# COSIMA/cice4

Measured on AMD Instinct MI355X. Metric: EVP subcycles/sec, higher is better.
Workload: dtype f64; 1 GPU; gx1-size 320x384 rectangular synthetic grid, full ice cover, ncat=5, ndte=120; nx_global=320, ny_global=384, ndte=120, decomposition=1x1 j-slabs, one block per GPU, subcycles_in_the_most_common_launch=120, metrics_recomputed_from_HTN_HTE=True, active_T_cells=121980, active_U_cells=121280

## Files before the change

cice4_amd/csrc/evp.hip:

```cpp
#include "evp.h"

#include <algorithm>
#include <array>
#include <cmath>
#include <cstdio>
#include <cstdlib>
#include <chrono>
#include <cstring>
#include <thread>

namespace cice {

using namespace K;

#ifdef CICE4_AMD_AUSCOM
__constant__ double cosw = 1.0, sinw = 0.0, dragw = dragio * rhow;
__constant__ int ocnslope = 0;

void evp_set_namelist(double cosw_, double sinw_, double dragio_, int use_ocnslope) {
  const double dragw_ = dragio_ * rhow;
  const int os = use_ocnslope != 0;
  CICE_HIP(hipMemcpyToSymbol(HIP_SYMBOL(cosw), &cosw_, 8));
  CICE_HIP(hipMemcpyToSymbol(HIP_SYMBOL(sinw), &sinw_, 8));
  CICE_HIP(hipMemcpyToSymbol(HIP_SYMBOL(dragw), &dragw_, 8));
// ... 89 lines not shown
  const double ssigm1 = (m1 + m3) * p055, ssigm2 = (m2 + m4) * p055;
  const double ssig12n = t1 + t2, ssig12s = t3 + t4, ssig12e = t1 + t4, ssig12w = t2 + t3;
  const double ssig121 = (t1 + t3) * p111, ssig122 = (t2 + t4) * p111;
  const double csigpne = p111 * p1 + ssigp2 + p027 * p3;
  const double csigpnw = p111 * p2 + ssigp1 + p027 * p4;
  const double csigpsw = p111 * p3 + ssigp2 + p027 * p1;
  const double csigpse = p111 * p4 + ssigp1 + p027 * p2;
  const double csigmne = p111 * m1 + ssigm2 + p027 * m3;
  const double csigmnw = p111 * m2 + ssigm1 + p027 * m4;
  const double csigmsw = p111 * m3 + ssigm2 + p027 * m1;
  const double csigmse = p111 * m4 + ssigm1 + p027 * m2;
  const double csig12ne = p222 * t1 + ssig122 + p055 * t3;
  const double csig12nw = p222 * t2 + ssig121 + p055 * t4;
  const double csig12sw = p222 * t3 + ssig122 + p055 * t1;
  const double csig12se = p222 * t4 + ssig121 + p055 * t2;
  const double str12ew = p5 * Dxt * (p333 * ssig12e + p166 * ssig12w);
  const double str12we = p5 * Dxt * (p333 * ssig12w + p166 * ssig12e);
  const double str12ns = p5 * Dyt * (p333 * ssig12n + p166 * ssig12s);
  const double str12sn = p5 * Dyt * (p333 * ssig12s + p166 * ssig12n);
  double strp_tmp = p25 * Dyt * (p333 * ssigpn + p166 * ssigps);
  double strm_tmp = p25 * Dyt * (p333 * ssigmn + p166 * ssigms);
  o.str[0] = -strp_tmp - strm_tmp - str12ew + Dxhy * (-csigpne + csigmne) + Dyhx * csig12ne;
  o.str[1] = strp_tmp + strm_tmp - str12we + Dxhy * (-csigpnw + csigmnw) + Dyhx * csig12nw;
  strp_tmp = p25 * Dyt * (p333 * ssigps + p166 * ssigpn);
  strm_tmp = p25 * Dyt * (p333 * ssigms + p166 * ssigmn);
  o.str[2] = -strp_tmp - strm_tmp + str12ew + Dxhy * (-csigpse + csigmse) + Dyhx * csig12se;
  o.str[3] = strp_tmp + strm_tmp + str12we + Dxhy * (-csigpsw + csigmsw) + Dyhx * csig12sw;
  strp_tmp = p25 * Dxt * (p333 * ssigpe + p166 * ssigpw);
  strm_tmp = p25 * Dxt * (p333 * ssigme + p166 * ssigmw);
  o.str[4] = -strp_tmp + strm_tmp - str12ns - Dyhx * (csigpne + csigmne) + Dxhy * csig12ne;
  o.str[5] = strp_tmp - strm_tmp - str12sn - Dyhx * (csigpse + csigmse) + Dxhy * csig12se;
  strp_tmp = p25 * Dxt * (p333 * ssigpw + p166 * ssigpe);
  strm_tmp = p25 * Dxt * (p333 * ssigmw + p166 * ssigme);
  o.str[6] = -strp_tmp + strm_tmp + str12ns - Dyhx * (csigpnw + csigmnw) + Dxhy * csig12nw;
  o.str[7] = strp_tmp - strm_tmp + str12sn - Dyhx * (csigpsw + csigmsw) + Dxhy * csig12sw;
}

__device__ __forceinline__ void water_of(double uo, double vo, double fmv, double& wx, double& wy) {
#ifdef CICE4_AMD_AUSCOM
  const double sg = __builtin_signbit(fmv) ? -1.0 : 1.0;
  wx = uo * cosw - vo * sinw * sg;
  wy = vo * cosw + uo * sinw * sg;
#else
  (void)fmv;
  wx = uo * cosw - vo * sinw;
  wy = vo * cosw + uo * sinw;
#endif
}

struct StepuOut {
  double u, v, strintx, strinty, taux, tauy;
};

__device__ __forceinline__ void stepu_cell(double uold, double vold, double Aiu, double Uocn,
                                           double Vocn, double Waterx, double Watery, double Forcex,
                                           double Forcey, double Umassdtei, double Fm, double Uarear,
                                           double sx, double sy, StepuOut& o) {
  const double du = Uocn - uold, dv = Vocn - vold;
  const double vrel = Aiu * dragw * sqrt(du * du + dv * dv);
  o.taux = vrel * Waterx;
  o.tauy = vrel * Watery;
  const double cca = Umassdtei + vrel * cosw;
#ifdef CICE4_AMD_AUSCOM
  const double ccb = Fm < 0.0 ? Fm - vrel * sinw : Fm + vrel * sinw;
#else
  const double ccb = Fm + vrel * sinw;
#endif
  const double ab2 = cca * cca + ccb * ccb;
  o.strintx = Uarear * sx;
  o.strinty = Uarear * sy;
  const double cc1 = o.strintx + Forcex + o.taux + Umassdtei * uold;
  const double cc2 = o.strinty + Forcey + o.tauy + Umassdtei * vold;
  o.u = (cca * cc1 + ccb * cc2) / ab2;
  o.v = (cca * cc2 - ccb * cc1) / ab2;
}

}

struct SubArgs {
  EvpScalars sc;
  int nx, ny, tiles_x, tiles_y, nblocks;
  int diag_jmin;
  int carry_top;
  int ew_cyclic;
  size_t n;
  const int32_t* __restrict__ ring_slot;
  const int32_t* __restrict__ fwd;
  const int32_t* __restrict__ blk;
  const int32_t* __restrict__ icetmask;
  const int32_t* __restrict__ iceumask;
  const double* __restrict__ u_in;
  const double* __restrict__ v_in;
  double* __restrict__ u_out;
  double* __restrict__ v_out;
  const double* __restrict__ sig_in;
  double* __restrict__ sig_out;
  const double* sig_in_p[12];
  double* sig_out_p[12];
  const double *__restrict__ dxt, *__restrict__ dyt, *__restrict__ dxhy, *__restrict__ dyhx,
      *__restrict__ cxp, *__restrict__ cyp, *__restrict__ cxm, *__restrict__ cym,
      *__restrict__ tarear, *__restrict__ tinyarea, *__restrict__ strength;
  const double *__restrict__ HTN, *__restrict__ HTE;
  const double *__restrict__ aiu, *__restrict__ uocn, *__restrict__ vocn, *__restrict__ waterx,
      *__restrict__ watery, *__restrict__ forcex, *__restrict__ forcey, *__restrict__ umassdtei,
      *__restrict__ fm, *__restrict__ uarear;
  double *__restrict__ divu, *__restrict__ rdg_conv, *__restrict__ rdg_shear, *__restrict__ shear,
      *__restrict__ prs_sig, *__restrict__ strintx, *__restrict__ strinty, *__restrict__ strocnx,
      *__restrict__ strocny;
};

namespace {


__device__ __forceinline__ double up1(double x) {
  int lo = __double2loint(x), hi = __double2hiint(x);
  lo = __builtin_amdgcn_update_dpp(lo, lo, 0x138, 0xf, 0xf, false);
  hi = __builtin_amdgcn_update_dpp(hi, hi, 0x138, 0xf, 0xf, false);
  return __hiloint2double(hi, lo);
}
__device__ __forceinline__ double down1(double x) {
  int lo = __double2loint(x), hi = __double2hiint(x);
  lo = __builtin_amdgcn_update_dpp(lo, lo, 0x130, 0xf, 0xf, false);
  hi = __builtin_amdgcn_update_dpp(hi, hi, 0x130, 0xf, 0xf, false);
  return __hiloint2double(hi, lo);
}

#ifndef SKEW_OPAQUE_STRIDE
#define SKEW_OPAQUE_STRIDE 1
#endif
#ifndef SKEW_TRIM
#define SKEW_TRIM 1
#endif
#ifndef SKEW_LOADPRIO
#define SKEW_LOADPRIO 1
#endif
#ifndef SKEW_TPASS
#define SKEW_TPASS 1
#endif
#ifndef SKEW_WIDE
#define SKEW_WIDE 1
#endif
#if !defined(CICE4_AMD_EXPERIMENTS) || !defined(SKEW_EARLY)
#undef SKEW_EARLY
#define SKEW_EARLY 0
#endif
__device__ __forceinline__ double up1z(double x) {
  int lo = __double2loint(x), hi = __double2hiint(x);
  lo = __builtin_amdgcn_update_dpp(0, lo, 0x138, 0xf, 0xf, true);
  hi = __builtin_amdgcn_update_dpp(0, hi, 0x138, 0xf, 0xf, true);
  return __hiloint2double(hi, lo);
}
__device__ __forceinline__ double down1z(double x) {
  int lo = __double2loint(x), hi = __double2hiint(x);
  lo = __builtin_amdgcn_update_dpp(0, lo, 0x130, 0xf, 0xf, true);
  hi = __builtin_amdgcn_update_dpp(0, hi, 0x130, 0xf, 0xf, true);
  return __hiloint2double(hi, lo);
}

constexpr int TX = 64;

struct UIn {
  double aiu, uocn, vocn, waterx, watery, forcex, forcey, umassdtei, fm, uarear;
};

template <bool DERIVE>
__device__ __forceinline__ void load_uin(const SubArgs& a, size_t q, UIn& x) {
  x.aiu = a.aiu[q]; x.uocn = a.uocn[q]; x.vocn = a.vocn[q];
  if (!DERIVE) {
    x.waterx = a.waterx[q];
    x.watery = a.watery[q];
  }
  x.forcex = a.forcex[q]; x.forcey = a.forcey[q];
  x.umassdtei = a.umassdtei[q]; x.fm = a.fm[q]; x.uarear = a.uarear[q];
  if (DERIVE) water_of(x.uocn, x.vocn, x.fm, x.waterx, x.watery);
}

template <bool LAST>
__device__ __forceinline__ void stepu_store(const SubArgs& a, const UIn& x, size_t q, int i, int j,
                                            int ilo, int ihi, int jlo, int jhi, double uold,
                                            double vold, double sx, double sy) {
  StepuOut r;
  stepu_cell(uold, vold, x.aiu, x.uocn, x.vocn, x.waterx, x.watery, x.forcex, x.forcey, x.umassdtei,
             x.fm, x.uarear, sx, sy, r);
  a.u_out[q] = r.u;
  a.v_out[q] = r.v;
  if (LAST && j >= a.diag_jmin) {
    a.strintx[q] = r.strintx;
    a.strinty[q] = r.strinty;
    a.strocnx[q] = r.taux;
    a.strocny[q] = r.tauy;
  }
  if (a.ring_slot && (i == ilo || i == ihi || j == jlo || j == jhi)) {
    const int slot = a.ring_slot[q];
    if (slot >= 0) {
#pragma unroll
      for (int k = 0; k < 3; ++k) {
        const int d = a.fwd[3 * slot + k];
        if (d >= 0) {
          a.u_out[d] = r.u;
          a.v_out[d] = r.v;
        }
      }
    }
  }
}

template <int W, int R, bool LAST, bool DAMP, bool DERIVE>
__global__ __launch_bounds__(64 * W, 4) void k_subcycle(const SubArgs a) {
// ... 924 lines not shown
    PHASE(2)
    __syncthreads();
    PHASE(3)
  }
  if (!ra) break;
  }
  stamp_at(sa.stamps, 1);
#ifdef CICE4_AMD_STAMPS
  ph_[6] = (long long)__builtin_amdgcn_s_getreg(20 | (31 << 11));
  ph_[7] = (long long)__builtin_amdgcn_s_getreg(4 | (31 << 11));
  if (sa.phases && lx == 0)
    for (int i_ = 0; i_ < 8; ++i_) sa.phases[8 * ((size_t)blockIdx.x * K + k) + i_] = ph_[i_];
#endif
  if (sa.dbg && threadIdx.x == 0) sa.dbg[2 * blockIdx.x + 1] = wall_clock64();
}

constexpr int RES_MAXDEP = 16;
constexpr int RES_NPEER = 8;
constexpr int RES_STRIDE = 32;

struct ResArgs {
  SubArgs a;
  int nsub, last;
  unsigned epoch0;
  unsigned* prog;
  unsigned* abort_flag;
  const int32_t* deps;
  double* xu[2];
  long long spin_ticks;
  const int32_t* rslot;
  const int32_t* rfwd;
  double* pxu[RES_NPEER][2];
  unsigned pn[RES_NPEER];
  unsigned* prp[RES_NPEER];
  const unsigned* rprog;
  const int32_t* pub;
  const int32_t* fslot;
  const int32_t* ffwd;
  const int32_t* ftab;
  double* xraw[2];
  unsigned* prog2;
  const int32_t* deps2;
  long long* stamps;
  long long* phases;
  int prio_mode;
  int prio_div;
  int prio_top;
  const int32_t* tile_map;
  const int32_t* src;
  void* xg;
  unsigned xg_half;
  void* xgr;
  int poll_delay, poll_sleep;
  int fake_ew;
};
enum { F_LO = 1, F_HI = 2, F_NEG = 4, F_SELF = 8, F_MIRROR = 16 };

__device__ __forceinline__ double ld_agent(const double* base, unsigned off) {
  return __hip_atomic_load((double*)((char*)const_cast<double*>(base) + off), __ATOMIC_RELAXED, __HIP_MEMORY_SCOPE_AGENT);
}
__device__ __forceinline__ void st_agent(double* base, unsigned off, double v) {
  __hip_atomic_store((double*)((char*)base + off), v, __ATOMIC_RELAXED, __HIP_MEMORY_SCOPE_AGENT);
}

__device__ __forceinline__ double ld_sys(const double* base, unsigned off) {
  return __hip_atomic_load((double*)((char*)const_cast<double*>(base) + off), __ATOMIC_RELAXED, __HIP_MEMORY_SCOPE_SYSTEM);
}
__device__ __forceinline__ void st_sys(double* base, unsigned off, double v) {
  __hip_atomic_store((double*)((char*)base + off), v, __ATOMIC_RELAXED, __HIP_MEMORY_SCOPE_SYSTEM);
}

typedef unsigned u32x4 __attribute__((ext_vector_type(4)));
__device__ __forceinline__ void st_gran(__amdgpu_buffer_rsrc_t rs, unsigned off, unsigned soff, double x, unsigned tag) {
  u32x4 g;
  g.x = (unsigned)__double2loint(x); g.y = tag; g.z = (unsigned)__double2hiint(x); g.w = tag;
  __builtin_amdgcn_raw_buffer_store_b128(g, rs, (int)off, (int)soff, 16);
  asm volatile("s_nop 1" : : "v"(g) : "memory");
}
__device__ __forceinline__ u32x4 ld_gran(__amdgpu_buffer_rsrc_t rs, unsigned off, unsigned soff) {
  return __builtin_amdgcn_raw_buffer_load_b128(rs, (int)off, (int)soff, 16);
}
#ifdef CICE4_AMD_STAMPS
__device__ __forceinline__ unsigned gran_tag(unsigned epoch) { return (epoch << 16) | ((unsigned)wall_clock64() & 0xffffu); }
__device__ __forceinline__ bool gran_ok(const u32x4& a, const u32x4& b, unsigned tag) {
  return ((a.y ^ tag) >> 16) == 0 && a.w == a.y && b.y == a.y && b.w == a.y;
}
#else
__device__ __forceinline__ unsigned gran_tag(unsigned epoch) { return epoch; }
__device__ __forceinline__ bool gran_ok(const u32x4& a, const u32x4& b, unsigned tag) {
  return a.y == tag && a.w == tag && b.y == tag && b.w == tag;
}
#endif
__device__ __forceinline__ double gran_val(const u32x4& a) { return __hiloint2double((int)a.z, (int)a.x); }

__global__ __launch_bounds__(1024) void k_res_choose_map(int nt, int tiles_x, int tiles_y, int W, int nx, int ny, int per_xcd,
                                                         int force, const int32_t* __restrict__ blk,
                                                         const int32_t* __restrict__ tmk, const int32_t* __restrict__ umk,
                                                         int32_t* __restrict__ out, unsigned* __restrict__ cover_word) {
  __shared__ int s_ice[1024];
  __shared__ int s_cnt[2][256];
  __shared__ int s_max[2];
  const int t = threadIdx.x;
  if (t < 256) s_cnt[0][t] = s_cnt[1][t] = 0;
  if (t < 2) s_max[t] = 0;
  int ice = 0;
  if (t < nt) {
    const int per_blk = tiles_x * tiles_y, b = t / per_blk, rem = t - b * per_blk, tyi = rem / tiles_x, txi = rem - tyi * tiles_x;
// ... 125 lines not shown
          for (int c = 0; c < 4; ++c) rf[c] = r.rfwd[4 * rs + c];
        }
      }
#pragma unroll
      for (int c = 0; c < 4; ++c) s_rfd[w][c][lx] = rf[c];
      edge = edge || rf[0] >= 0;
    }
    if (FOLD) {
      if (uown) {
        const int rs = r.fslot[q];
        if (rs >= 0) {
#pragma unroll
          for (int c = 0; c < 4; ++c) rfr[c] = r.ffwd[4 * rs + c];
        }
      }
      edge = edge || rfr[0] >= 0;
    }
  }
  const bool topc = FOLD && uown && j == jhi;
  const bool toptile = FOLD && j0 + (W - 2) >= jhi;
  int fpad = -1, fmode = 0;
  if (topc) {
    fpad = r.ftab[2 * q];
    fmode = r.ftab[2 * q + 1];
    edge = true;
  }
  const bool rghost = PEER && ok && !uown && r.rslot[q] == -2;
  bool need_f = false, need_s = false;
  const unsigned qg = (unsigned)q * 32u, nxg = (unsigned)nx * 32u;
  unsigned offA = qg, offB = qg - nxg;
  bool nA = false, nB = false;
  int lw = -1, lq = -1;
  bool lw_a = false, lq_a = false;
  if (GRAN) {
    auto produced = [&](size_t cell) { return r.src[cell] >= 0; };
    need_f = foreign && produced(q);
    need_s = south_h && produced(q - nx);
    nA = need_f;
    nB = need_s;
    const bool nw_ = west_h && produced(q - 1), nq_ = west_h && produced(q - nx - 1);
    const unsigned q0g = (unsigned)__builtin_amdgcn_readfirstlane((int)qg);
    const unsigned long long want_w = __ballot(nw_), want_q = __ballot(nq_);
    auto lend = [&](unsigned off, int& lane, bool& in_a) {
      const unsigned long long fa = __ballot(!nA && lx != 0), fb = __ballot(!nB && lx != 0);
      in_a = fa != 0;
      lane = (int)__builtin_ctzll(in_a ? fa : (fb ? fb : 1ull));
      if (lx == lane && lane != 0) {
        if (in_a) { offA = off; nA = true; }
        else { offB = off; nB = true; }
      }
    };
    if (want_w) lend(q0g - 32u, lw, lw_a);
    if (want_q) lend(q0g - nxg - 32u, lq, lq_a);
    if (r.fake_ew && w > 0 && w < W - 1) {
      nA = nB = false;
      lw = lq = -1;
    }
  }
  StressOut o;
  StepuOut ro{};

  s_uv[w][0][lx] = un;
  s_uv[w][1][lx] = vn;
  __syncthreads();
  if (PEER) {
    const unsigned begun = r.epoch0 + 1u;
    if (threadIdx.x == 0)
      __hip_atomic_store(r.prog + (size_t)tile * RES_STRIDE, begun, __ATOMIC_RELAXED, __HIP_MEMORY_SCOPE_AGENT);
    if (threadIdx.x < RES_NPEER && s_pub[threadIdx.x])
      __hip_atomic_store(r.prp[threadIdx.x] + (size_t)tile * RES_STRIDE, begun, __ATOMIC_RELAXED, __HIP_MEMORY_SCOPE_SYSTEM);
  }
  stamp_at(r.stamps, 0);
  PHASE_DECL
  const int gen = r.prio_div > 0 ? min(2, (int)(blockIdx.x >> 3) / r.prio_div) : 0;
  if (!GRAN && r.prio_mode == 1) {
    if (gen == 0) __builtin_amdgcn_s_setprio(3);
    else if (gen == 1) __builtin_amdgcn_s_setprio(2);
    else __builtin_amdgcn_s_setprio(0);
  }
  if constexpr (GRAN) {
#ifndef GRAN_COPIES
#define GRAN_COPIES 2
#endif
    const __amdgpu_buffer_rsrc_t rs = __builtin_amdgcn_make_buffer_rsrc(r.xg, 0, GRAN_COPIES * r.xg_half, 0x00020000);
    const bool prio_work = r.prio_mode >= 5;
    const bool chain_hi = r.prio_mode == 5 && (w == 0 || w >= W - 2);
    auto prio_wait = [&]() { if (prio_work) __builtin_amdgcn_s_setprio(0); };
    auto prio_compute = [&]() {
      if (prio_work) {
        if (chain_hi) __builtin_amdgcn_s_setprio(3);
        else __builtin_amdgcn_s_setprio(2);
      }
    };
    auto wait_row = [&](int* flag, int want) -> bool {
      long long t0 = 0;
      for (int it = 0;; ++it) {
        if (__hip_atomic_load(flag, __ATOMIC_RELAXED, __HIP_MEMORY_SCOPE_WORKGROUP) >= want) break;
        if (it == 0) prio_wait();
        if (__hip_atomic_load(&s_abort, __ATOMIC_RELAXED, __HIP_MEMORY_SCOPE_WORKGROUP)) return false;
        if (it == 0) t0 = wall_clock64();
        else if ((it & 63) == 0 && wall_clock64() - t0 > 2 * r.spin_ticks) {
          if (lx == 0 && __hip_atomic_exchange(r.abort_flag, 1u, __ATOMIC_RELAXED, __HIP_MEMORY_SCOPE_AGENT) == 0u) {
            r.abort_flag[1] = 5u; r.abort_flag[2] = (unsigned)tile; r.abort_flag[3] = 0u;
            r.abort_flag[4] = (unsigned)w; r.abort_flag[5] = (unsigned)want; r.abort_flag[6] = 0u;
          }
          __hip_atomic_store(&s_abort, 1, __ATOMIC_RELAXED, __HIP_MEMORY_SCOPE_WORKGROUP);
          return false;
        }
        __builtin_amdgcn_s_sleep(1);
      }
      asm volatile("" ::: "memory");
      prio_compute();
      return true;
    };
    auto post_row = [&](int* flag, int value) {
      asm volatile("s_waitcnt lgkmcnt(0)" ::: "memory");
      if (lx == 0) __hip_atomic_store(flag, value, __ATOMIC_RELAXED, __HIP_MEMORY_SCOPE_WORKGROUP);
    };
    TRACE_DECL
    const bool chain = w == 0 || w >= W - 2;
    if (r.prio_mode == 1) {
      if (chain) __builtin_amdgcn_s_setprio(3);
      else __builtin_amdgcn_s_setprio(1);
    }
    prio_compute();
#pragma clang loop unroll(disable)
    for (int k = 0; k < r.nsub; ++k) {
      const bool lastk = r.last && k == r.nsub - 1;
      if (r.prio_mode == 2) {
        const int p = (k + gen) % 3;
        if (p == 0) __builtin_amdgcn_s_setprio(3);
        else if (p == 1) __builtin_amdgcn_s_setprio(1);
        else __builtin_amdgcn_s_setprio(0);
      } else if (r.prio_mode == 3) {
        int behind = 0, level = 0;
        for (int o = w & 3; o < W - 1; o += 4)
          if (o != w) {
            const int done = __hip_atomic_load(&s_uf[o], __ATOMIC_RELAXED, __HIP_MEMORY_SCOPE_WORKGROUP);
            behind += done < k;
            level += done == k;
          }
        if (behind) __builtin_amdgcn_s_setprio(0);
        else if (level) __builtin_amdgcn_s_setprio(2);
        else __builtin_amdgcn_s_setprio(3);
      } else if (r.prio_mode == 4) {
        const int p = (k + gen) & 3;
        if (p == 0) __builtin_amdgcn_s_setprio(3);
        else if (p == 1) __builtin_amdgcn_s_setprio(2);
        else if (p == 2) __builtin_amdgcn_s_setprio(1);
        else __builtin_amdgcn_s_setprio(0);
      }
      PHASE(7)
      TRACE(0)
      if (w > 0) {
        if (!wait_row(&s_uf[w - 1], k)) return;
        if (!south_h) {
          us = s_uv[w - 1][0][lx];
          vs = s_uv[w - 1][1][lx];
        }
      }
      TRACE(1)
      double uw = up1(un), vw = up1(vn), usw = up1(us), vsw = up1(vs);
      if (lx == 0) {
        uw = uwh;
        vw = vwh;
        usw = uswh;
        vsw = vswh;
      }
#pragma unroll
      for (int c = 0; c < 8; ++c) o.str[c] = c0;
      if (tact) {
        const double Dxt = s_m[w][0][lx], Dyt = s_m[w][1][lx], Dxhy = s_m[w][2][lx], Dyhx = s_m[w][3][lx],
                     Cxp = s_m[w][5][lx], Cyp = s_m[w][6][lx], Cxm = s_m[w][7][lx], Cym = s_m[w][8][lx],
                     Tiny = s_m[w][9][lx];
        stress_cell<true, DAMP>(a.sc, un, uw, usw, us, vn, vw, vsw, vs, Dxt, Dyt, Dxhy, Dyhx, Cxp, Cyp, Cxm, Cym,
                                lastk ? a.tarear[q] : c0, Tiny, s_m[w][4][lx], s, o, lastk);
      }
      const double e1 = down1(o.str[1]), e3 = down1(o.str[3]), e6 = down1(o.str[6]), e7 = down1(o.str[7]);
      if (w > 0) {
        s_edge[w][0][lx] = o.str[2];
        s_edge[w][1][lx] = e3;
        s_edge[w][2][lx] = o.str[5];
        s_edge[w][3][lx] = e7;
      }
      post_row(&s_sf[w], k + 1);
      TRACE(2)
      PHASE(0)
      if (w < W - 1) {
        if (!wait_row(&s_sf[w + 1], k + 1)) return;
        TRACE(3)
        PHASE(1)
        if (uact) {
          const double sx = o.str[0] + e1 + s_edge[w + 1][0][lx] + s_edge[w + 1][1][lx];
          const double sy = o.str[4] + s_edge[w + 1][2][lx] + e6 + s_edge[w + 1][3][lx];
          const double uocn = s_x[w][1][lx], vocn = s_x[w][2][lx];
          double wx, wy;
          water_of(uocn, vocn, s_x[w][6][lx], wx, wy);
          stepu_cell(un, vn, s_x[w][0][lx], uocn, vocn, wx, wy,
                     s_x[w][3][lx], s_x[w][4][lx], s_x[w][5][lx], s_x[w][6][lx], s_x[w][7][lx], sx, sy, ro);
          un = ro.u;
          vn = ro.v;
        }
      }
      const unsigned par = (unsigned)(k & (GRAN_COPIES - 1)) * r.xg_half;
      if constexpr (FOLD) {
        if (__any(topc)) {
          const __amdgpu_buffer_rsrc_t rsr = __builtin_amdgcn_make_buffer_rsrc(r.xgr, 0, 4 * r.xg_half, 0x00020000);
          const unsigned tag2 = gran_tag(r.epoch0 + (unsigned)k + 1u);
          const unsigned par4 = (unsigned)(k & 3) * r.xg_half;
          if (topc) {
            st_gran(rsr, qg, par4, un, tag2);
            st_gran(rsr, qg + 16u, par4, vn, tag2);
          }
          bool pp = topc && fmode != 0 && !(fmode & F_SELF);
          u32x4 p0 = {0u, 0u, 0u, 0u}, p1 = p0;
          if (__any(pp)) {
            prio_wait();
            const long long t0 = wall_clock64();
            int it = 0;
            while (true) {
              if (pp) { p0 = ld_gran(rsr, (unsigned)fpad * 32u, par4); p1 = ld_gran(rsr, (unsigned)fpad * 32u + 16u, par4); }
              if (pp && gran_ok(p0, p1, tag2)) pp = false;
              if (!__any(pp)) break;
              asm volatile("" ::: "memory");
              int bad = __hip_atomic_load(&s_abort, __ATOMIC_RELAXED, __HIP_MEMORY_SCOPE_WORKGROUP);
              if (!bad && (++it & 7) == 0) bad = (int)__hip_atomic_load(r.abort_flag, __ATOMIC_RELAXED, __HIP_MEMORY_SCOPE_AGENT);
              if (!bad && wall_clock64() - t0 > r.spin_ticks) {
                if (lx == (int)__builtin_ctzll(__ballot(pp)) &&
                    __hip_atomic_exchange(r.abort_flag, 1u, __ATOMIC_RELAXED, __HIP_MEMORY_SCOPE_AGENT) == 0u) {
                  r.abort_flag[1] = 6u; r.abort_flag[2] = (unsigned)tile; r.abort_flag[3] = (unsigned)k;
                  r.abort_flag[4] = (unsigned)w; r.abort_flag[5] = (unsigned)lx; r.abort_flag[6] = tag2;
                }
                bad = 1;
              }
              if (__any(bad)) {
                __hip_atomic_store(&s_abort, 1, __ATOMIC_RELAXED, __HIP_MEMORY_SCOPE_WORKGROUP);
                return;
              }
              __builtin_amdgcn_s_sleep(1);
            }
            prio_compute();
          }
          if (topc && fmode) {
            if (fmode & F_SELF) {
              un = -un;
              vn = -vn;
            } else {
              const double pu = gran_val(p0), pv = gran_val(p1);
              if (fmode & F_MIRROR) {
                un = (fmode & F_NEG) ? -pu : pu;
                vn = (fmode & F_NEG) ? -pv : pv;
              } else {
                const double u1 = (fmode & F_LO) ? un : pu, u2 = (fmode & F_LO) ? pu : un;
                const double v1 = (fmode & F_LO) ? vn : pv, v2 = (fmode & F_LO) ? pv : vn;
                const double xu_ = 0.5 * (u1 + (-u2)), xv_ = 0.5 * (v1 + (-v2));
                un = (fmode & F_NEG) ? -xu_ : xu_;
                vn = (fmode & F_NEG) ? -xv_ : xv_;
              }
            }
          }
        }
      }
      if (k + 1 == r.nsub) break;
      const unsigned tag = gran_tag(r.epoch0 + (unsigned)k + 1u);
      if (edge) {
        st_gran(rs, qg, par, un, tag);
        st_gran(rs, qg + 16u, par, vn, tag);
#pragma unroll
        for (int c = 0; c < 3; ++c) {
          const int fd = s_fd[w][c][lx];
          if (fd >= 0) {
            st_gran(rs, (unsigned)fd * 32u, par, un, tag);
            st_gran(rs, (unsigned)fd * 32u + 16u, par, vn, tag);
          }
        }
        if (FOLD) {
#pragma unroll
          for (int c = 0; c < 4; ++c) {
            const int rf = rfr[c];
            if (rf >= 0) {
              const bool neg = (rf >> 30) & 1;
              const unsigned ro = (unsigned)(rf & 0x3fffffff) * 32u;
              st_gran(rs, ro, par, neg ? -un : un, tag);
              st_gran(rs, ro + 16u, par, neg ? -vn : vn, tag);
            }
          }
        }
      }
      s_uv[w][0][lx] = un;
      s_uv[w][1][lx] = vn;
      post_row(&s_uf[w], k + 1);
      TRACE(4)
      PHASE(2)
      bool pa = nA, pb = nB;
      if (__any(pa || pb)) {
        prio_wait();
        const long long t0 = wall_clock64();
        int it = 0;
        for (int d = 0; d < r.poll_delay; ++d) __builtin_amdgcn_s_sleep(8);
        u32x4 a0 = {0u, 0u, 0u, 0u}, a1 = a0, b0 = a0, b1 = a0;
        while (true) {
          if (pa) { a0 = ld_gran(rs, offA, par); a1 = ld_gran(rs, offA + 16u, par); }
          if (pb) { b0 = ld_gran(rs, offB, par); b1 = ld_gran(rs, offB + 16u, par); }
          if (pa && gran_ok(a0, a1, tag)) pa = false;
          if (pb && gran_ok(b0, b1, tag)) pb = false;
          PHASE_COUNT(4, 1)
          if (it == 0) { PHASE(3) }
          if (!__any(pa || pb)) break;
          asm volatile("" ::: "memory");
          int bad = __hip_atomic_load(&s_abort, __ATOMIC_RELAXED, __HIP_MEMORY_SCOPE_WORKGROUP);
          if (!bad && (++it & 7) == 0) bad = (int)__hip_atomic_load(r.abort_flag, __ATOMIC_RELAXED, __HIP_MEMORY_SCOPE_AGENT);
          if (!bad && wall_clock64() - t0 > r.spin_ticks) {
            if (lx == (int)__builtin_ctzll(__ballot(pa || pb)) &&
                __hip_atomic_exchange(r.abort_flag, 1u, __ATOMIC_RELAXED, __HIP_MEMORY_SCOPE_AGENT) == 0u) {
              r.abort_flag[1] = 4u; r.abort_flag[2] = (unsigned)tile; r.abort_flag[3] = (unsigned)k;
              r.abort_flag[4] = (unsigned)w; r.abort_flag[5] = (unsigned)lx | (pa ? 256u : 0u) | (pb ? 512u : 0u);
              r.abort_flag[6] = tag;
            }
            bad = 1;
          }
          if (__any(bad)) {
            __hip_atomic_store(&s_abort, 1, __ATOMIC_RELAXED, __HIP_MEMORY_SCOPE_WORKGROUP);
            return;
          }
          __builtin_amdgcn_s_sleep(1);
          for (int d = 0; d < r.poll_sleep; ++d) __builtin_amdgcn_s_sleep(8);
        }
#ifdef CICE4_AMD_STAMPS
        {
          const unsigned now = (unsigned)wall_clock64() & 0xffffu;
          const unsigned ta = nA ? ((now - a0.y) & 0xffffu) : 0u, tb = nB ? ((now - b0.y) & 0xffffu) : 0u;
          PHASE_COUNT(5, (long long)(ta > tb ? ta : tb))
        }
#endif
        const double au = gran_val(a0), av = gran_val(a1), bu = gran_val(b0), bv = gran_val(b1);
        if (need_f) { un = au; vn = av; }
        if (need_s) { us = bu; vs = bv; }
        if (lw >= 0) {
          const double xu_ = __shfl(lw_a ? au : bu, lw), xv_ = __shfl(lw_a ? av : bv, lw);
          if (lx == 0) { uwh = xu_; vwh = xv_; }
        }
        if (lq >= 0) {
          const double xu_ = __shfl(lq_a ? au : bu, lq), xv_ = __shfl(lq_a ? av : bv, lq);
          if (lx == 0) { uswh = xu_; vswh = xv_; }
        }
        prio_compute();
      }
      TRACE(5)
      PHASE(6)
    }
  } else {
#pragma clang loop unroll(disable)
  for (int k = 0; k < r.nsub; ++k) {
    const bool lastk = r.last && k == r.nsub - 1;
    if (FOLD && toptile && r.prio_top) {
      __builtin_amdgcn_s_setprio(3);
    } else if (r.prio_mode == 2) {
      const int p = (k + gen) % 3;
      if (p == 0) __builtin_amdgcn_s_setprio(3);
      else if (p == 1) __builtin_amdgcn_s_setprio(1);
      else __builtin_amdgcn_s_setprio(0);
    }
    PHASE_DRAIN
    PHASE(7)
    if (!south_h && w > 0) {
      us = s_uv[w - 1][0][lx];
      vs = s_uv[w - 1][1][lx];
    }
    double uw = up1(un), vw = up1(vn), usw = up1(us), vsw = up1(vs);
    if (lx == 0) {
      uw = uwh;
      vw = vwh;
      usw = uswh;
      vsw = vswh;
    }
#pragma unroll
    for (int c = 0; c < 8; ++c) o.str[c] = c0;
    if (tact) {
      const double Dxt = s_m[w][0][lx], Dyt = s_m[w][1][lx], Dxhy = s_m[w][2][lx], Dyhx = s_m[w][3][lx],
                   Cxp = s_m[w][5][lx], Cyp = s_m[w][6][lx], Cxm = s_m[w][7][lx], Cym = s_m[w][8][lx],
                   Tiny = s_m[w][9][lx];
      stress_cell<true, DAMP>(a.sc, un, uw, usw, us, vn, vw, vsw, vs, Dxt, Dyt, Dxhy, Dyhx, Cxp, Cyp, Cxm, Cym,
                              lastk ? a.tarear[q] : c0, Tiny, s_m[w][4][lx], s, o, lastk);
    }
    const double e1 = down1(o.str[1]), e3 = down1(o.str[3]), e6 = down1(o.str[6]), e7 = down1(o.str[7]);
    if (w > 0) {
      s_edge[w][0][lx] = o.str[2];
      s_edge[w][1][lx] = e3;
      s_edge[w][2][lx] = o.str[5];
      s_edge[w][3][lx] = e7;
    }
    PHASE(0)
    __syncthreads();
    PHASE(1)
    if (uact) {
      const double sx = o.str[0] + e1 + s_edge[w + 1][0][lx] + s_edge[w + 1][1][lx];
      const double sy = o.str[4] + s_edge[w + 1][2][lx] + e6 + s_edge[w + 1][3][lx];
      const double uocn = s_x[w][1][lx], vocn = s_x[w][2][lx];
      double wx, wy;
      water_of(uocn, vocn, s_x[w][6][lx], wx, wy);
      stepu_cell(un, vn, s_x[w][0][lx], uocn, vocn, wx, wy,
                 s_x[w][3][lx], s_x[w][4][lx], s_x[w][5][lx], s_x[w][6][lx], s_x[w][7][lx], sx, sy, ro);
      un = ro.u;
      vn = ro.v;
    }
    if (FOLD && toptile) {
      double* xr = r.xraw[k & 1];
      if (topc) {
        st_agent(xr, qb, un);
        st_agent(xr + a.n, qb, vn);
      }
      asm volatile("s_waitcnt vmcnt(0)" ::: "memory");
      __syncthreads();
      const unsigned target2 = r.epoch0 + (unsigned)k + 1u;
      if (threadIdx.x == 0)
        __hip_atomic_store(r.prog2 + (size_t)tile * RES_STRIDE, target2, __ATOMIC_RELAXED, __HIP_MEMORY_SCOPE_AGENT);
      if (w == 0) {
        const int dep = lx < 4 ? r.deps2[tile * 4 + lx] : -1;
        bool have = dep < 0;
        int bad = 0;
        const long long t0 = wall_clock64();
        while (true) {
          if (!have)
            have = (int)(__hip_atomic_load(r.prog2 + (size_t)dep * RES_STRIDE, __ATOMIC_RELAXED, __HIP_MEMORY_SCOPE_AGENT) - target2) >= 0;
          if (__all(have)) break;
          const unsigned long long miss = __ballot(!have);
          if (lx == 0) {
            bad = (int)__hip_atomic_load(r.abort_flag, __ATOMIC_RELAXED, __HIP_MEMORY_SCOPE_AGENT);
            if (!bad && wall_clock64() - t0 > r.spin_ticks) {
              if (__hip_atomic_exchange(r.abort_flag, 1u, __ATOMIC_RELAXED, __HIP_MEMORY_SCOPE_AGENT) == 0u) {
                r.abort_flag[1] = 3u; r.abort_flag[2] = (unsigned)tile; r.abort_flag[3] = (unsigned)k;
                r.abort_flag[4] = (unsigned)miss; r.abort_flag[5] = 0u; r.abort_flag[6] = target2;
              }
              bad = 1;
            }
          }
          bad = __shfl(bad, 0);
          if (bad) break;
          __builtin_amdgcn_s_sleep(2);
        }
        if (lx == 0) s_abort = bad;
      }
      __syncthreads();
      if (s_abort) return;
      if (topc && fmode) {
        if (fmode & F_SELF) {
          un = -un;
          vn = -vn;
        } else {
          const double pu = ld_agent(xr, (unsigned)fpad * 8u), pv = ld_agent(xr + a.n, (unsigned)fpad * 8u);
          if (fmode & F_MIRROR) {
            un = (fmode & F_NEG) ? -pu : pu;
            vn = (fmode & F_NEG) ? -pv : pv;
          } else {
            const double u1 = (fmode & F_LO) ? un : pu, u2 = (fmode & F_LO) ? pu : un;
// ... 3048 lines not shown
  if (res_epoch > 0x70000000u) {
    CICE_REQUIRE(!peer, "resident EVP loop across ranks: progress epoch exhausted (re-create the context)");
    res_prog.zero(stream);
    if (res_prog2.p) res_prog2.zero(stream);
    if (res_xg.p) res_xg.zero(stream);
    if (res_xgr.p) res_xgr.zero(stream);
    res_epoch = 0;
  }
  ResArgs r{};
  r.a = make_args();
  r.a.tiles_x = ((dom.nx_block - 2) + (TX - 1) - 1) / (TX - 1);
  r.a.tiles_y = ((dom.ny_block - 2) + (W - 1) - 1) / (W - 1);
  r.nsub = nsub;
  r.last = (ksub0 + nsub - 1 == sc.ndte) ? 1 : 0;
  r.epoch0 = res_epoch;
  r.prog = res_prog.p;
  r.abort_flag = res_prog.p + (size_t)res_tiles * RES_STRIDE;
  r.deps = res_deps.p;
  r.xu[0] = res_xu[0].p;
  r.xu[1] = res_xu[1].p;
  r.spin_ticks = (long long)res_spin_us * 100;
  if (halo.has_fold()) {
    r.fslot = res_fslot.p;
    r.ffwd = res_ffwd.p;
    r.ftab = res_ftab.p;
    r.xraw[0] = res_xraw[0].p;
    r.xraw[1] = res_xraw[1].p;
    r.prog2 = res_prog2.p;
    r.deps2 = res_deps2.p;
  }
  if (peer) {
    r.rslot = res_rslot.p;
    r.rfwd = res_rfwd.p;
    r.rprog = res_rprog.p;
    r.pub = res_pub.p;
    for (int sd = 0; sd < RES_NPEER; ++sd) {
      r.pxu[sd][0] = peers[sd].xu[0];
      r.pxu[sd][1] = peers[sd].xu[1];
      r.pn[sd] = peers[sd].n;
      r.prp[sd] = peers[sd].rprog ? peers[sd].rprog + (size_t)peer_back[(size_t)sd] * RP_MAX * RES_STRIDE : nullptr;
    }
  }
  const bool dense = !peer && resident_dense();
  const bool gran = !peer && granules_on() && !dense && res_xg.p && res_src.p && (!halo.has_fold() || res_xgr.p);
  if (gran) {
    r.src = res_src.p;
    r.xg = res_xg.p;
    r.xg_half = (unsigned)(n * 32);
    r.xgr = res_xgr.p;
    static const int pd = [] { const char* e = std::getenv("CICE4_AMD_RESIDENT_POLL_DELAY"); return e ? std::atoi(e) : 2; }();
    static const int ps = [] { const char* e = std::getenv("CICE4_AMD_RESIDENT_POLL_SLEEP"); return e ? std::atoi(e) : 0; }();
    r.poll_delay = pd;
    r.poll_sleep = ps;
    static const int fk = [] { const char* e = std::getenv("CICE4_AMD_RESIDENT_FAKE_EW"); return e ? std::atoi(e) : 0; }();
    r.fake_ew = fk;
  } else {
    for (int k = 0; k < 2; ++k)
      CICE_HIP(hipMemcpyAsync(res_xu[k].p, uv[cur].p, 2 * n * 8, hipMemcpyDeviceToDevice, stream));
  }
  const dim3 g(8 * ((res_tiles + 7) / 8));
  const bool damp = sc.evp_damping != 0;
  {
    const int ncu = device_cus();
    const int per_cu = resident_occupancy(W, damp, peer);
    if ((long long)per_cu * ncu < (long long)g.x) {
      std::fprintf(stderr, "cice4_amd: resident EVP loop not used: %u workgroups of %d wavefronts, the device holds %d x %d "
                           "of this kernel\n", g.x, W, per_cu, ncu);
      if (dense) res_level = 1;
      else resident_failed = true;
      return false;
    }
  }
  r.prio_mode = gran ? (res_prio == 2 ? 4 : res_prio) : (dense ? std::min(res_prio, 2) : 0);
  {
    static const bool top = [] { const char* e = std::getenv("CICE4_AMD_RESIDENT_PRIO_TOP"); return !(e && e[0] == '0'); }();
    r.prio_top = dense && top ? 1 : 0;
  }
  r.tile_map = nullptr;
  if (!peer && !halo.has_fold() && g.x <= 1024) {
    if (res_map.n == 0) { res_map.alloc(4); res_map_stale = true; }
    if (res_map_stale) {
      static const int force = [] { const char* e = std::getenv("CICE4_AMD_RESIDENT_MAP"); return e ? std::atoi(e) : -1; }();
      const int ncu = device_cus();
      hipLaunchKernelGGL(k_res_choose_map, dim3(1), dim3(1024), 0, stream, r.a.tiles_x * r.a.tiles_y * r.a.nblocks, r.a.tiles_x,
                         r.a.tiles_y, W, dom.nx_block, dom.ny_block, std::max(1, ncu / 8), res_map_opt >= 0 ? res_map_opt : force,
                         (const int32_t*)blk.p, (const int32_t*)icetmask.p, (const int32_t*)iceumask.p, res_map.p, r.abort_flag + 7);
      res_map_stale = false;
    }
    r.tile_map = res_map.p;
  }
  {
    const int ncu = device_cus();
    r.prio_div = std::max(1, ncu / 8);
  }
  r.stamps = stamp_buffer(3 * (size_t)g.x + 600);
  r.phases = r.stamps ? r.stamps + 4 * (size_t)g.x : nullptr;
  if (res_time_it) CICE_HIP(hipEventRecord(res_t0, stream));
  switch (W) {
    case 4: launch_res<4>(r, damp, peer, g, stream); break;
    case 6: launch_res<6>(r, damp, peer, g, stream); break;
    case 8: launch_res<8>(r, damp, peer, g, stream); break;
    case 11: launch_res<11>(r, damp, peer, g, stream); break;
    case 12: launch_res<12>(r, damp, peer, g, stream); break;
    default: throw Error{CICE_EINVAL, "resident_waves must be 4, 6, 8, 11 or 12"};
  }
  if (res_time_it) {
    CICE_HIP(hipEventRecord(res_t1, stream));
    res_timed = true;
  }
  if (const hipError_t le = hipGetLastError(); le != hipSuccess) {
    std::fprintf(stderr, "cice4_amd: resident EVP loop could not be launched (%s); this range runs as one launch per pair "
                         "of subcycles and so do later ones\n", hipGetErrorString(le));
    CICE_REQUIRE(!peer, "resident EVP loop across ranks: launch failed on this rank");
    resident_failed = true;
    return false;
  }
  if (!res_why) CICE_HIP(hipHostMalloc((void**)&res_why, (RES_RING + 1) * 8 * sizeof(unsigned), hipHostMallocDefault));
  if (res_defer && !peer) {
    const int slot = (int)res_pending.size();
    CICE_REQUIRE(slot < RES_RING, "resident EVP loop: more launches pending than records");
    CICE_HIP(hipMemcpyAsync(res_why + 8 * (size_t)slot, r.abort_flag, 8 * sizeof(unsigned), hipMemcpyDeviceToHost, stream));
    res_pending.push_back(ResPending{ksub0, nsub, cur, flips, copies_identical, dense, r.tile_map != nullptr, res_epoch, slot});
    res_epoch += (unsigned)nsub;
    cur = 1 - cur;
    ++flips;
    copies_identical = false;
// ... 326 lines not shown
```

Measured before the change: 210,000 subcycles/s.

## Split stepu into head/tail to overlap with neighbor wait, and scalarize resident-loop control

Splits the momentum update into a head part, which depends only on old velocities and forcing, and a tail part that needs the stress divergence. The head now runs before waiting on the neighbouring wavefront's stress flag, so its arithmetic overlaps that wait. The change also hoists the metric loads from shared memory, makes poll and wait conditions wave-uniform via readfirstlane, replaces the lane-0 halo select with a DPP bound_ctrl source, and takes halo values with readlane instead of shfl. Experimental priority modes and the fake-EW path are compiled out unless a build flag is set, at the cost of more live registers across the wait.

```diff
diff --git a/cice4_amd/csrc/evp.hip b/cice4_amd/csrc/evp.hip
--- a/cice4_amd/csrc/evp.hip
+++ b/cice4_amd/csrc/evp.hip
@@ -165,27 +165,43 @@
   double u, v, strintx, strinty, taux, tauy;
 };
 
+struct StepuHead {
+  double taux, tauy, cca, ccb, ab2, mu, mv;
+};
+__device__ __forceinline__ void stepu_head(double uold, double vold, double Aiu, double Uocn, double Vocn,
+                                           double Waterx, double Watery, double Umassdtei, double Fm, StepuHead& h) {
+  const double du = Uocn - uold, dv = Vocn - vold;
+  const double vrel = Aiu * dragw * sqrt(du * du + dv * dv);
+  h.taux = vrel * Waterx;
+  h.tauy = vrel * Watery;
+  h.cca = Umassdtei + vrel * cosw;
+#ifdef CICE4_AMD_AUSCOM
+  h.ccb = Fm < 0.0 ? Fm - vrel * sinw : Fm + vrel * sinw;
+#else
+  h.ccb = Fm + vrel * sinw;
+#endif
+  h.ab2 = h.cca * h.cca + h.ccb * h.ccb;
+  h.mu = Umassdtei * uold;
+  h.mv = Umassdtei * vold;
+}
+__device__ __forceinline__ void stepu_tail(const StepuHead& h, double Forcex, double Forcey, double Uarear, double sx,
+                                           double sy, StepuOut& o) {
+  o.taux = h.taux;
+  o.tauy = h.tauy;
+  o.strintx = Uarear * sx;
+  o.strinty = Uarear * sy;
+  const double cc1 = o.strintx + Forcex + h.taux + h.mu;
+  const double cc2 = o.strinty + Forcey + h.tauy + h.mv;
+  o.u = (h.cca * cc1 + h.ccb * cc2) / h.ab2;
+  o.v = (h.cca * cc2 - h.ccb * cc1) / h.ab2;
+}
 __device__ __forceinline__ void stepu_cell(double uold, double vold, double Aiu, double Uocn,
                                            double Vocn, double Waterx, double Watery, double Forcex,
                                            double Forcey, double Umassdtei, double Fm, double Uarear,
                                            double sx, double sy, StepuOut& o) {
-  const double du = Uocn - uold, dv = Vocn - vold;
-  const double vrel = Aiu * dragw * sqrt(du * du + dv * dv);
-  o.taux = vrel * Waterx;
-  o.tauy = vrel * Watery;
-  const double cca = Umassdtei + vrel * cosw;
-#ifdef CICE4_AMD_AUSCOM
-  const double ccb = Fm < 0.0 ? Fm - vrel * sinw : Fm + vrel * sinw;
-#else
-  const double ccb = Fm + vrel * sinw;
-#endif
-  const double ab2 = cca * cca + ccb * ccb;
-  o.strintx = Uarear * sx;
-  o.strinty = Uarear * sy;
-  const double cc1 = o.strintx + Forcex + o.taux + Umassdtei * uold;
-  const double cc2 = o.strinty + Forcey + o.tauy + Umassdtei * vold;
-  o.u = (cca * cc1 + ccb * cc2) / ab2;
-  o.v = (cca * cc2 - ccb * cc1) / ab2;
+  StepuHead h;
+  stepu_head(uold, vold, Aiu, Uocn, Vocn, Waterx, Watery, Umassdtei, Fm, h);
+  stepu_tail(h, Forcex, Forcey, Uarear, sx, sy, o);
 }
 
 }
@@ -267,6 +283,13 @@
   int lo = __double2loint(x), hi = __double2hiint(x);
   lo = __builtin_amdgcn_update_dpp(0, lo, 0x130, 0xf, 0xf, true);
   hi = __builtin_amdgcn_update_dpp(0, hi, 0x130, 0xf, 0xf, true);
+  return __hiloint2double(hi, lo);
+}
+
+__device__ __forceinline__ double up1_first(double x, double first) {
+  int lo = __double2loint(x), hi = __double2hiint(x);
+  lo = __builtin_amdgcn_update_dpp(__double2loint(first), lo, 0x138, 0xf, 0xf, false);
+  hi = __builtin_amdgcn_update_dpp(__double2hiint(first), hi, 0x138, 0xf, 0xf, false);
   return __hiloint2double(hi, lo);
 }
 
@@ -1297,7 +1320,9 @@
   unsigned xg_half;
   void* xgr;
   int poll_delay, poll_sleep;
+#ifdef CICE4_AMD_EXPERIMENTS
   int fake_ew;
+#endif
 };
 enum { F_LO = 1, F_HI = 2, F_NEG = 4, F_SELF = 8, F_MIRROR = 16 };
 
@@ -1529,10 +1554,12 @@
     };
     if (want_w) lend(q0g - 32u, lw, lw_a);
     if (want_q) lend(q0g - nxg - 32u, lq, lq_a);
+#ifdef CICE4_AMD_EXPERIMENTS
     if (r.fake_ew && w > 0 && w < W - 1) {
       nA = nB = false;
       lw = lq = -1;
     }
+#endif
   }
   StressOut o;
   StepuOut ro{};
@@ -1560,6 +1587,7 @@
 #define GRAN_COPIES 2
 #endif
     const __amdgpu_buffer_rsrc_t rs = __builtin_amdgcn_make_buffer_rsrc(r.xg, 0, GRAN_COPIES * r.xg_half, 0x00020000);
+#ifdef CICE4_AMD_EXPERIMENTS
     const bool prio_work = r.prio_mode >= 5;
     const bool chain_hi = r.prio_mode == 5 && (w == 0 || w >= W - 2);
     auto prio_wait = [&]() { if (prio_work) __builtin_amdgcn_s_setprio(0); };
@@ -1569,12 +1597,17 @@
         else __builtin_amdgcn_s_setprio(2);
       }
     };
+#else
+    auto prio_wait = []() {};
+    auto prio_compute = []() {};
+#endif
+    const int rot = r.prio_mode == 4 ? gen : -1;
     auto wait_row = [&](int* flag, int want) -> bool {
       long long t0 = 0;
       for (int it = 0;; ++it) {
-        if (__hip_atomic_load(flag, __ATOMIC_RELAXED, __HIP_MEMORY_SCOPE_WORKGROUP) >= want) break;
+        if (__builtin_amdgcn_readfirstlane(__hip_atomic_load(flag, __ATOMIC_RELAXED, __HIP_MEMORY_SCOPE_WORKGROUP)) >= want) break;
         if (it == 0) prio_wait();
-        if (__hip_atomic_load(&s_abort, __ATOMIC_RELAXED, __HIP_MEMORY_SCOPE_WORKGROUP)) return false;
+        if (__builtin_amdgcn_readfirstlane(__hip_atomic_load(&s_abort, __ATOMIC_RELAXED, __HIP_MEMORY_SCOPE_WORKGROUP))) return false;
         if (it == 0) t0 = wall_clock64();
         else if ((it & 63) == 0 && wall_clock64() - t0 > 2 * r.spin_ticks) {
           if (lx == 0 && __hip_atomic_exchange(r.abort_flag, 1u, __ATOMIC_RELAXED, __HIP_MEMORY_SCOPE_AGENT) == 0u) {
@@ -1595,21 +1628,37 @@
       if (lx == 0) __hip_atomic_store(flag, value, __ATOMIC_RELAXED, __HIP_MEMORY_SCOPE_WORKGROUP);
     };
     TRACE_DECL
+#ifdef CICE4_AMD_EXPERIMENTS
     const bool chain = w == 0 || w >= W - 2;
     if (r.prio_mode == 1) {
       if (chain) __builtin_amdgcn_s_setprio(3);
       else __builtin_amdgcn_s_setprio(1);
     }
+#endif
     prio_compute();
+    const int lend_w = __builtin_amdgcn_readfirstlane(lw < 0 ? -1 : (lw | (lw_a ? 64 : 0)));
+    const int lend_q = __builtin_amdgcn_readfirstlane(lq < 0 ? -1 : (lq | (lq_a ? 64 : 0)));
+    const int polls = __builtin_amdgcn_readfirstlane((int)__any(nA || nB));
+    auto word = [](int x) { asm volatile("" : "+s"(x)); return x; };
+    auto take = [](const u32x4& ga, const u32x4& gb, int code) {
+      const bool in_a = (code & 64) != 0;
+      const int lane = code & 63;
+      return __hiloint2double(__builtin_amdgcn_readlane((int)(in_a ? ga.z : gb.z), lane),
+                              __builtin_amdgcn_readlane((int)(in_a ? ga.x : gb.x), lane));
+    };
 #pragma clang loop unroll(disable)
     for (int k = 0; k < r.nsub; ++k) {
       const bool lastk = r.last && k == r.nsub - 1;
-      if (r.prio_mode == 2) {
-        const int p = (k + gen) % 3;
-        if (p == 0) __builtin_amdgcn_s_setprio(3);
-        else if (p == 1) __builtin_amdgcn_s_setprio(1);
-        else __builtin_amdgcn_s_setprio(0);
-      } else if (r.prio_mode == 3) {
+      if (rot >= 0) {
+        switch ((k + rot) & 3) {
+          case 0: __builtin_amdgcn_s_setprio(3); break;
+          case 1: __builtin_amdgcn_s_setprio(2); break;
+          case 2: __builtin_amdgcn_s_setprio(1); break;
+          default: __builtin_amdgcn_s_setprio(0); break;
+        }
+      }
+#ifdef CICE4_AMD_EXPERIMENTS
+      if (r.prio_mode == 3) {
         int behind = 0, level = 0;
         for (int o = w & 3; o < W - 1; o += 4)
           if (o != w) {
@@ -1620,15 +1669,13 @@
         if (behind) __builtin_amdgcn_s_setprio(0);
         else if (level) __builtin_amdgcn_s_setprio(2);
         else __builtin_amdgcn_s_setprio(3);
-      } else if (r.prio_mode == 4) {
-        const int p = (k + gen) & 3;
-        if (p == 0) __builtin_amdgcn_s_setprio(3);
-        else if (p == 1) __builtin_amdgcn_s_setprio(2);
-        else if (p == 2) __builtin_amdgcn_s_setprio(1);
-        else __builtin_amdgcn_s_setprio(0);
-      }
+      }
+#endif
       PHASE(7)
       TRACE(0)
+      double m[10];
+#pragma unroll
+      for (int c = 0; c < 10; ++c) m[c] = s_m[w][c][lx];
       if (w > 0) {
         if (!wait_row(&s_uf[w - 1], k)) return;
         if (!south_h) {
@@ -1637,23 +1684,14 @@
         }
       }
       TRACE(1)
-      double uw = up1(un), vw = up1(vn), usw = up1(us), vsw = up1(vs);
-      if (lx == 0) {
-        uw = uwh;
-        vw = vwh;
-        usw = uswh;
-        vsw = vswh;
-      }
+      const double uw = up1_first(un, uwh), vw = up1_first(vn, vwh), usw = up1_first(us, uswh), vsw = up1_first(vs, vswh);
 #pragma unroll
       for (int c = 0; c < 8; ++c) o.str[c] = c0;
       if (tact) {
-        const double Dxt = s_m[w][0][lx], Dyt = s_m[w][1][lx], Dxhy = s_m[w][2][lx], Dyhx = s_m[w][3][lx],
-                     Cxp = s_m[w][5][lx], Cyp = s_m[w][6][lx], Cxm = s_m[w][7][lx], Cym = s_m[w][8][lx],
-                     Tiny = s_m[w][9][lx];
-        stress_cell<true, DAMP>(a.sc, un, uw, usw, us, vn, vw, vsw, vs, Dxt, Dyt, Dxhy, Dyhx, Cxp, Cyp, Cxm, Cym,
-                                lastk ? a.tarear[q] : c0, Tiny, s_m[w][4][lx], s, o, lastk);
-      }
-      const double e1 = down1(o.str[1]), e3 = down1(o.str[3]), e6 = down1(o.str[6]), e7 = down1(o.str[7]);
+        stress_cell<true, DAMP>(a.sc, un, uw, usw, us, vn, vw, vsw, vs, m[0], m[1], m[2], m[3], m[5], m[6], m[7], m[8],
+                                lastk ? a.tarear[q] : c0, m[9], m[4], s, o, lastk);
+      }
+      const double e1 = down1z(o.str[1]), e3 = down1z(o.str[3]), e6 = down1z(o.str[6]), e7 = down1z(o.str[7]);
       if (w > 0) {
         s_edge[w][0][lx] = o.str[2];
         s_edge[w][1][lx] = e3;
@@ -1664,17 +1702,25 @@
       TRACE(2)
       PHASE(0)
       if (w < W - 1) {
+        StepuHead hd{};
+        double forcex = c0, forcey = c0, uarear = c0;
+        if (uact) {
+          const double uocn = s_x[w][1][lx], vocn = s_x[w][2][lx], fm = s_x[w][6][lx];
+          double wx, wy;
+          water_of(uocn, vocn, fm, wx, wy);
+          stepu_head(un, vn, s_x[w][0][lx], uocn, vocn, wx, wy, s_x[w][5][lx], fm, hd);
+          forcex = s_x[w][3][lx];
+          forcey = s_x[w][4][lx];
+          uarear = s_x[w][7][lx];
+        }
+        asm volatile("" : "+v"(hd.taux), "+v"(hd.tauy), "+v"(hd.cca), "+v"(hd.ccb), "+v"(hd.ab2), "+v"(hd.mu), "+v"(hd.mv));
         if (!wait_row(&s_sf[w + 1], k + 1)) return;
         TRACE(3)
         PHASE(1)
         if (uact) {
           const double sx = o.str[0] + e1 + s_edge[w + 1][0][lx] + s_edge[w + 1][1][lx];
           const double sy = o.str[4] + s_edge[w + 1][2][lx] + e6 + s_edge[w + 1][3][lx];
-          const double uocn = s_x[w][1][lx], vocn = s_x[w][2][lx];
-          double wx, wy;
-          water_of(uocn, vocn, s_x[w][6][lx], wx, wy);
-          stepu_cell(un, vn, s_x[w][0][lx], uocn, vocn, wx, wy,
-                     s_x[w][3][lx], s_x[w][4][lx], s_x[w][5][lx], s_x[w][6][lx], s_x[w][7][lx], sx, sy, ro);
+          stepu_tail(hd, forcex, forcey, uarear, sx, sy, ro);
           un = ro.u;
           vn = ro.v;
         }
@@ -1770,12 +1816,13 @@
       TRACE(4)
       PHASE(2)
       bool pa = nA, pb = nB;
-      if (__any(pa || pb)) {
+      if (polls) {
         prio_wait();
         const long long t0 = wall_clock64();
         int it = 0;
-        for (int d = 0; d < r.poll_delay; ++d) __builtin_amdgcn_s_sleep(8);
-        u32x4 a0 = {0u, 0u, 0u, 0u}, a1 = a0, b0 = a0, b1 = a0;
+        for (int d = word(r.poll_delay); d > 0; --d) __builtin_amdgcn_s_sleep(8);
+        u32x4 a0, a1, b0, b1;
+        asm volatile("" : "=v"(a0), "=v"(a1), "=v"(b0), "=v"(b1));
         while (true) {
           if (pa) { a0 = ld_gran(rs, offA, par); a1 = ld_gran(rs, offA + 16u, par); }
           if (pb) { b0 = ld_gran(rs, offB, par); b1 = ld_gran(rs, offB + 16u, par); }
@@ -1813,14 +1860,9 @@
         const double au = gran_val(a0), av = gran_val(a1), bu = gran_val(b0), bv = gran_val(b1);
         if (need_f) { un = au; vn = av; }
         if (need_s) { us = bu; vs = bv; }
-        if (lw >= 0) {
-          const double xu_ = __shfl(lw_a ? au : bu, lw), xv_ = __shfl(lw_a ? av : bv, lw);
-          if (lx == 0) { uwh = xu_; vwh = xv_; }
-        }
-        if (lq >= 0) {
-          const double xu_ = __shfl(lq_a ? au : bu, lq), xv_ = __shfl(lq_a ? av : bv, lq);
-          if (lx == 0) { uswh = xu_; vswh = xv_; }
-        }
+        const int cw = word(lend_w), cq = word(lend_q);
+        if (cw >= 0) { uwh = take(a0, b0, cw); vwh = take(a1, b1, cw); }
+        if (cq >= 0) { uswh = take(a0, b0, cq); vswh = take(a1, b1, cq); }
         prio_compute();
       }
       TRACE(5)
@@ -1844,13 +1886,7 @@
       us = s_uv[w - 1][0][lx];
       vs = s_uv[w - 1][1][lx];
     }
-    double uw = up1(un), vw = up1(vn), usw = up1(us), vsw = up1(vs);
-    if (lx == 0) {
-      uw = uwh;
-      vw = vwh;
-      usw = uswh;
-      vsw = vswh;
-    }
+    const double uw = up1_first(un, uwh), vw = up1_first(vn, vwh), usw = up1_first(us, uswh), vsw = up1_first(vs, vswh);
 #pragma unroll
     for (int c = 0; c < 8; ++c) o.str[c] = c0;
     if (tact) {
@@ -1860,7 +1896,7 @@
       stress_cell<true, DAMP>(a.sc, un, uw, usw, us, vn, vw, vsw, vs, Dxt, Dyt, Dxhy, Dyhx, Cxp, Cyp, Cxm, Cym,
                               lastk ? a.tarear[q] : c0, Tiny, s_m[w][4][lx], s, o, lastk);
     }
-    const double e1 = down1(o.str[1]), e3 = down1(o.str[3]), e6 = down1(o.str[6]), e7 = down1(o.str[7]);
+    const double e1 = down1z(o.str[1]), e3 = down1z(o.str[3]), e6 = down1z(o.str[6]), e7 = down1z(o.str[7]);
     if (w > 0) {
       s_edge[w][0][lx] = o.str[2];
       s_edge[w][1][lx] = e3;
@@ -1868,16 +1904,23 @@
       s_edge[w][3][lx] = e7;
     }
     PHASE(0)
+    StepuHead hd{};
+    double forcex = c0, forcey = c0, uarear = c0;
+    if (uact) {
+      const double uocn = s_x[w][1][lx], vocn = s_x[w][2][lx], fm = s_x[w][6][lx];
+      double wx, wy;
+      water_of(uocn, vocn, fm, wx, wy);
+      stepu_head(un, vn, s_x[w][0][lx], uocn, vocn, wx, wy, s_x[w][5][lx], fm, hd);
+      forcex = s_x[w][3][lx];
+      forcey = s_x[w][4][lx];
+      uarear = s_x[w][7][lx];
+    }
     __syncthreads();
     PHASE(1)
     if (uact) {
       const double sx = o.str[0] + e1 + s_edge[w + 1][0][lx] + s_edge[w + 1][1][lx];
       const double sy = o.str[4] + s_edge[w + 1][2][lx] + e6 + s_edge[w + 1][3][lx];
-      const double uocn = s_x[w][1][lx], vocn = s_x[w][2][lx];
-      double wx, wy;
-      water_of(uocn, vocn, s_x[w][6][lx], wx, wy);
-      stepu_cell(un, vn, s_x[w][0][lx], uocn, vocn, wx, wy,
-                 s_x[w][3][lx], s_x[w][4][lx], s_x[w][5][lx], s_x[w][6][lx], s_x[w][7][lx], sx, sy, ro);
+      stepu_tail(hd, forcex, forcey, uarear, sx, sy, ro);
       un = ro.u;
       vn = ro.v;
     }
@@ -5032,8 +5075,10 @@
     static const int ps = [] { const char* e = std::getenv("CICE4_AMD_RESIDENT_POLL_SLEEP"); return e ? std::atoi(e) : 0; }();
     r.poll_delay = pd;
     r.poll_sleep = ps;
+#ifdef CICE4_AMD_EXPERIMENTS
     static const int fk = [] { const char* e = std::getenv("CICE4_AMD_RESIDENT_FAKE_EW"); return e ? std::atoi(e) : 0; }();
     r.fake_ew = fk;
+#endif
   } else {
     for (int k = 0; k < 2; ++k)
       CICE_HIP(hipMemcpyAsync(res_xu[k].p, uv[cur].p, 2 * n * 8, hipMemcpyDeviceToDevice, stream));
@@ -5051,7 +5096,11 @@
       return false;
     }
   }
+#ifdef CICE4_AMD_EXPERIMENTS
   r.prio_mode = gran ? (res_prio == 2 ? 4 : res_prio) : (dense ? std::min(res_prio, 2) : 0);
+#else
+  r.prio_mode = gran ? (res_prio == 0 ? 0 : 4) : (dense ? std::min(res_prio, 2) : 0);
+#endif
   {
     static const bool top = [] { const char* e = std::getenv("CICE4_AMD_RESIDENT_PRIO_TOP"); return !(e && e[0] == '0'); }();
     r.prio_top = dense && top ? 1 : 0;
```

New measurement: 223,100 subcycles/s, median of 6. +6.2%, better.
